# nmndeep/Robust-Segmentation

Measured on AMD Instinct MI355X. Metric: SEA attack-iterations/sec (UperNet-CNX-T, 512x512), higher is better.
Workload: dtype f32 (frozen-weight GEMMs on the 16-bit matrix cores by operand splitting: fp16x2 (22 significant bits per operand, 3 MFMA products) forward, fp16x2 (22 significant bits per operand, 3 MFMA products) input gradient; fp32 storage and accumulate)

## Files before the change

### devtools/gemm_big_stamps.py

```python
#!/usr/bin/env python3
import ctypes as C
import os
import subprocess
import sys

ROOT = os.path.dirname(os.path.dirname(os.path.abspath(__file__)))
PKG = os.path.join(ROOT, "robust-segmentation_amd")
SO = os.path.join(ROOT, "devtools", "_knock", "libbigdiag.so")

if "--build" in sys.argv:
    os.makedirs(os.path.dirname(SO), exist_ok=True)
    subprocess.run(["/opt/rocm/bin/hipcc", "-O3", "-fPIC", "-shared", "-std=c++17", "--offload-arch=gfx950", "-fno-slp-vectorize",
                    "-DSEA_GEMM_BIG_DIAG", os.path.join(PKG, "csrc", "gemm_split_big.hip"), "-o", SO], check=True)
    print(SO)
    sys.exit(0)

sys.path[:0] = [ROOT, PKG]
import numpy as np
import torch
from semseg import _native as N

args = [a for a in sys.argv[1:] if not a.startswith("-")]
G, M, K, Nn = [int(v) for v in (args[:4] if len(args) >= 4 else (36, 8192, 512, 512))]
STEPS = next(([int(v) for v in a[8:].split(",")] for a in sys.argv if a.startswith("--steps=")), [0, 93, 186, 372, 690])
L = C.CDLL(SO)
L.sea_gemm_big_diag.restype = C.c_int
L.sea_gemm_big_diag.argtypes = [C.c_void_p, C.c_int64, C.c_void_p, C.c_void_p, C.c_int64, C.c_int, C.c_int, C.c_int, C.c_int,
                                C.c_int64, C.c_int64, C.c_int64, C.c_void_p, C.c_int, C.c_int, C.c_int, C.c_void_p, C.c_void_p]
A = torch.randn(G, M, K, device="cuda")
W = torch.randn(G, Nn, K, device="cuda") / K ** 0.5
Wp = N.gemm_split_pack(W, terms=22)
out = torch.empty(G, M, Nn, device="cuda")
amax = torch.empty(M, dtype=torch.int32, device="cuda")
N.lib().sea_absmax_bits(N._p(A[0]), K, M, K, 1, 0, 1, N._p(amax), N._stream())
TILES = G * ((M + 255) // 256) * (Nn // 256)
stamps = torch.zeros(TILES, 8, dtype=torch.int64, device="cuda")
CUS = torch.cuda.get_device_properties(0).multi_processor_count


def launch(ko, step, st=None):
    rc = L.sea_gemm_big_diag(A.data_ptr(), K, Wp.data.data_ptr(), out.data_ptr(), Nn, M, Nn, K, G, M * K, Wp.stride, M * Nn,
                             amax.data_ptr(), 1, ko, step, st.data_ptr() if st is not None else None, N._stream())
    assert rc == 0, rc


def timed(ko, step, reps=20):
    launch(ko, step)
    torch.cuda.synchronize()
    e0, e1 = torch.cuda.Event(enable_timing=True), torch.cuda.Event(enable_timing=True)
    e0.record()
    for _ in range(reps):
        launch(ko, step)
    e1.record()
    torch.cuda.synchronize()
    return e0.elapsed_time(e1) / reps * 1e3


def us(ticks):
    return np.asarray(ticks, dtype=np.float64) / 100.0


def warm(seconds=2.0):
    import time
    t0 = time.perf_counter()
    while time.perf_counter() - t0 < seconds:
        for _ in range(50):
            launch(0, 0)
        torch.cuda.synchronize()


def stamp_table(ko, step):
    warm(0.5)
    for i in range(10):
        launch(ko, step, stamps if i == 5 else None)
    torch.cuda.synchronize()
    s = stamps.cpu().numpy().astype(np.int64)
    t = s[:, :6] - s[:, 0].min()
    cu = ((s[:, 6] >> 32) & 0xf) * 256 + ((s[:, 6] >> 8) & 0xff)
    seg = {"entry -> first load (stagger wait)": t[:, 1] - t[:, 0], "first load -> first MFMA (prologue)": t[:, 2] - t[:, 1],
           "K loop": t[:, 3] - t[:, 2], "K loop end -> last store issued": t[:, 4] - t[:, 3],
           "last store issued -> drained": t[:, 5] - t[:, 4], "whole block": t[:, 5] - t[:, 0]}
    print(f"\nko={ko} step={step} ticks: {len(np.unique(cu))} distinct CUs, launch span {us(t[:, 5].max()):.1f} us\n")
    print("| segment (wave 0) | median us | p10 | p90 |\n|---|---|---|---|")
    for name, v in seg.items():
        print(f"| {name} | {np.median(us(v)):.2f} | {np.percentile(us(v), 10):.2f} | {np.percentile(us(v), 90):.2f} |")
    gaps, rounds = [], {}
    for c in np.unique(cu):
        rows = t[cu == c]
        rows = rows[np.argsort(rows[:, 0])]
        gaps += list(rows[1:, 0] - rows[:-1, 5])
        for r, row in enumerate(rows):
            rounds.setdefault(r, []).append(row)
    g = us(gaps)
    print(f"| block end -> successor's entry, same CU | {np.median(g):.2f} | {np.percentile(g, 10):.2f} | {np.percentile(g, 90):.2f} |")
    print("\n| round on its CU | blocks | K-loop end: p10-p90 span over CUs, us | median block us | median K loop us | median K loop end -> stores issued us |\n|---|---|---|---|---|---|")
    for r in sorted(rounds):
        rows = np.array(rounds[r])
        if len(rows) < 16:
            continue
        e = us(rows[:, 3])
        print(f"| {r} | {len(rows)} | {np.percentile(e, 90) - np.percentile(e, 10):.1f} | {np.median(us(rows[:, 5] - rows[:, 0])):.1f} |"
              f" {np.median(us(rows[:, 3] - rows[:, 2])):.1f} | {np.median(us(rows[:, 4] - rows[:, 3])):.2f} |")


print(f"## G={G} M={M} K={K} N={Nn}: {TILES} tiles, {CUS} CUs, {K // 32} K steps, C = {G * M * Nn * 4 / 1e6:.0f} MB")
warm()
stamp_table(0, 0)
stamp_table(0, 186)
stamp_table(1, 0)
stamp_table(64, 0)
warm(0.5)
print("\n| 20 launches back to back, median [min - max] of five rounds taken in turn | full kernel us | non-temporal C stores us | no C stores us |\n|---|---|---|---|")
res = {(ko, step): [] for step in STEPS for ko in (0, 64, 1)}
for _ in range(5):
    for key in res:
        res[key].append(timed(*key))
for step in STEPS:
    cells = " | ".join(f"{np.median(res[ko, step]):.1f} [{min(res[ko, step]):.1f} - {max(res[ko, step]):.1f}]" for ko in (0, 64, 1))
    print(f"| stagger step {step} ticks (spread {step * 8 / 100:.1f} us) | {cells} |", flush=True)
```

### robust-segmentation_amd/csrc/gemm_split_big.hip

```cpp
#include "gemm_split.h"

namespace sea {

#ifdef SEA_GEMM_BIG_DIAG
struct BigDiag {
  int first_round, step_ticks;
  unsigned long long* stamps;
};
#define SEA_BIG_DIAG_PARAM , const BigDiag dg
#define SEA_BIG_DIAG_ARG , dg
#define SEA_BIG_STAMP(i) do { if constexpr (STAMP) { __builtin_amdgcn_sched_barrier(0); stamp[i] = __builtin_amdgcn_s_memrealtime(); __builtin_amdgcn_sched_barrier(0); } } while (0)
#else
#define SEA_BIG_DIAG_PARAM
#define SEA_BIG_DIAG_ARG
#define SEA_BIG_STAMP(i) do {} while (0)
#endif

template <bool F16, int WM, int WN, int TN, int PRO, int DEPTH, int KO = 0, bool STAMP = false>
__global__ __launch_bounds__(64 * WM * WN) void gemm_split_big_kernel(const GemmSplitArgs p SEA_BIG_DIAG_PARAM) {
  static_assert(WM * WN == 8, "eight waves, two per SIMD");
  constexpr int TERMS = 2;
  constexpr int MI = 2;
  constexpr int NT = 64 * WM * WN;
  constexpr int RP = NT / 8;
  constexpr int BM = 32 * MI * WM, WT = 32 * TN, BN = WT * WN;
  constexpr int IMG_A = BM * 64, IMG_W = BN * 64;
  constexpr int STAGE = TERMS * (IMG_A + IMG_W);
  constexpr int NA = BM / RP;
  constexpr int NWT = BN * 4 / NT, NW = TERMS * NWT;
  constexpr int SLOTS = 3 * MI * TN;
  constexpr int UNIT_EVERY = SLOTS / (3 * NA);
  constexpr bool HAS_T = (PRO == 1 || PRO == 3);
  static_assert(STAGE == 65536 && SLOTS % (3 * NA) == 0 && NW + 2 <= SLOTS, "configuration");
  extern __shared__ __attribute__((aligned(16))) char smem[];
  float* const row_sc = (float*)(smem + 2 * STAGE);
  float* const row_inv = row_sc + BM;

  const int M = p.M, N = p.N, K = p.K, Npad = p.Npad;
  const int64_t lda = p.lda, ldc = p.ldc;
  const int logical = (int)(blockIdx.x & 7) * p.per_xcd + (int)(blockIdx.x >> 3);
  if ((int)(blockIdx.x >> 3) >= p.per_xcd || logical >= p.total) return;
  const int nb = logical % p.nblocks;
  const int t2 = logical / p.nblocks;
  const int mb = t2 % p.mblocks;
  const int g = t2 / p.mblocks;
  const int m0 = mb * BM, n0 = nb * BN;
#ifdef SEA_GEMM_BIG_DIAG
  [[maybe_unused]] uint64_t stamp[6] = {};
  SEA_BIG_STAMP(0);
  if ((int)blockIdx.x < dg.first_round) {
    const uint32_t want = (uint32_t)(t2 % 8) * (uint32_t)dg.step_ticks;
    const uint32_t trips = (want >> 3) + 16;
    const uint64_t t0 = __builtin_amdgcn_s_memrealtime();
    for (uint32_t it = 0; it < trips && (uint32_t)(__builtin_amdgcn_s_memrealtime() - t0) < want; ++it) __builtin_amdgcn_s_sleep(8);
  }
  SEA_BIG_STAMP(1);
#endif
  const float* const w_inv = F16 ? (const float*)((const char*)p.w_inv + (int64_t)g * p.strideW) : nullptr;

  const int tid = threadIdx.x, lane = tid & 63, wave = tid >> 6;
  const int wm = wave / WN, wn = wave % WN;
  const int r = lane & 31, h = lane >> 5;
  const int q = tid & 7, arow = tid >> 3;

  const char* const Abase = (const char*)(p.A + (int64_t)g * p.strideA);
  const char* const Tbase = HAS_T ? (const char*)(p.a_gelu_grad_of + (int64_t)g * p.strideA) : nullptr;
  const float* const bias = p.bias;
  const int nkb = K / GS_BK;
  const char* const Wbase = p.W + (int64_t)g * p.strideW + (int64_t)n0 * 64;
  const int64_t w_term = (int64_t)Npad * 64, w_kb = (int64_t)TERMS * w_term;
  const uint32_t woff = (uint32_t)tid * 16;
  const uint32_t a_bytes = (uint32_t)((((int64_t)(M - 1)) * lda + K) * 4);
  const uint32_t w_bytes = (uint32_t)((int64_t)nkb * w_kb - (int64_t)n0 * 64);

  float a_sc[NA];
#pragma unroll
  for (int i = 0; i < NA; ++i) a_sc[i] = 1.f;
  const uint32_t aoff0 = (uint32_t)(((int64_t)(m0 + arow) * lda + 4 * q) * 4);
  const uint32_t a_wr0 = (uint32_t)(arow * 64 + swz<false>(arow, q >> 1) + (q & 1) * 8);
  const int wrow0 = tid >> 2;
  const uint32_t w_wr0 = (uint32_t)(TERMS * IMG_A + wrow0 * 64 + swz<false>(wrow0, tid & 3));
  const int a_row_step = (int)(RP * lda * 4);
  const int ra = wm * 32 * MI + r, rb = wn * WT + r;
  const uint32_t a_rd = (uint32_t)(ra * 64 + swz<false>(ra, h));
  const uint32_t b_rd = (uint32_t)(TERMS * IMG_A + rb * 64 + swz<false>(rb, h));

  struct Tile {
    f32x4 a[NA];
    f32x4 t[HAS_T ? NA : 1];
    u32x4 w[NW];
  };
  Tile R0 = {}, R1 = {};
  auto fetch_a = [&](Tile& R, int kb) __attribute__((always_inline)) {
    f32x4 (&Ra)[NA] = R.a;
    f32x4 (&Rt)[HAS_T ? NA : 1] = R.t;
    const int live = kb < nkb ? (int)a_bytes : 0;
    const __amdgpu_buffer_rsrc_t rs = __builtin_amdgcn_make_buffer_rsrc((void*)Abase, 0, live, 0x00020000);
#pragma unroll
    for (int i = 0; i < NA; ++i)
      Ra[i] = __builtin_bit_cast(f32x4, __builtin_amdgcn_raw_buffer_load_b128(
          rs, (int)((m0 + arow + RP * i < M) ? aoff0 : a_bytes), kb * (GS_BK * 4) + i * a_row_step, 0));
    if constexpr (HAS_T) {
      const __amdgpu_buffer_rsrc_t rt = __builtin_amdgcn_make_buffer_rsrc((void*)Tbase, 0, live, 0x00020000);
#pragma unroll
      for (int i = 0; i < NA; ++i)
        Rt[i] = __builtin_bit_cast(f32x4, __builtin_amdgcn_raw_buffer_load_b128(
            rt, (int)((m0 + arow + RP * i < M) ? aoff0 : a_bytes), kb * (GS_BK * 4) + i * a_row_step, 0));
    }
  };
  auto fetch_w = [&](Tile& R, int kb) __attribute__((always_inline)) {
    u32x4 (&Rw)[NW] = R.w;
    const __amdgpu_buffer_rsrc_t rs = __builtin_amdgcn_make_buffer_rsrc((void*)Wbase, 0, kb < nkb ? (int)w_bytes : 0, 0x00020000);
#pragma unroll
    for (int i = 0; i < NW; ++i)
      Rw[i] = __builtin_bit_cast(u32x4, __builtin_amdgcn_raw_buffer_load_b128(
                                            rs, (int)woff, kb * (int)w_kb + (i / NWT) * (int)w_term + (i % NWT) * (16 * NT), 0));
  };
  auto write_w = [&](Tile& R, int i, char* stage) __attribute__((always_inline)) {
    *(u32x4*)(stage + w_wr0 + (i / NWT) * IMG_W + (i % NWT) * (16 * NT)) = R.w[i];
  };

  f32x4 sv;
  uint32_t hi_a, hi_b;
  auto unit_a = [&](Tile& R, int i, int part, char* stage) __attribute__((always_inline)) {
    f32x4 (&Rt)[HAS_T ? NA : 1] = R.t;
    if (part == 0) {
      f32x4 v = R.a[i];
      if constexpr (PRO == 1) {
#pragma unroll
        for (int e = 0; e < 4; ++e) v[e] *= gelu_grad_f(Rt[i][e]);
      }
      if constexpr (PRO == 2) {
#pragma unroll
        for (int e = 0; e < 4; ++e) v[e] = gelu_f(v[e]);
      }
      if constexpr (PRO == 3) {
#pragma unroll
        for (int e = 0; e < 4; ++e) v[e] = Rt[i][e] > 0.f ? v[e] : 0.f;
      }
      if constexpr (F16) {
#pragma unroll
        for (int e = 0; e < 4; ++e) v[e] *= a_sc[i];
        hi_a = pack_f16(v[0], v[1]);
        hi_b = pack_f16(v[2], v[3]);
      } else {
        hi_a = pack_bf16(v[0], v[1]);
        hi_b = pack_bf16(v[2], v[3]);
      }
      sv = v;
    } else if (part == 1) {
      if constexpr (F16) {
        const f32x2 f0 = __builtin_convertvector(__builtin_bit_cast(f16x2, hi_a), f32x2);
        const f32x2 f1 = __builtin_convertvector(__builtin_bit_cast(f16x2, hi_b), f32x2);
        sv[0] -= f0[0];
        sv[1] -= f0[1];
        sv[2] -= f1[0];
        sv[3] -= f1[1];
      } else {
#pragma clang fp contract(off)
        sv[0] -= __uint_as_float(hi_a << 16);
        sv[1] -= __uint_as_float(hi_a & 0xffff0000u);
        sv[2] -= __uint_as_float(hi_b << 16);
        sv[3] -= __uint_as_float(hi_b & 0xffff0000u);
      }
    } else {
      *(u32x2*)(stage + a_wr0 + 64 * RP * i) = u32x2{hi_a, hi_b};
      const u32x2 mid = F16 ? u32x2{pack_f16(sv[0], sv[1]), pack_f16(sv[2], sv[3])}
                            : u32x2{pack_bf16(sv[0], sv[1]), pack_bf16(sv[2], sv[3])};
      *(u32x2*)(stage + IMG_A + a_wr0 + 64 * RP * i) = mid;
    }
  };

  bf16x8 fa[MI][TERMS], fb[TN][TERMS];
  auto read_a = [&](const char* stage, int s) __attribute__((always_inline)) {
#pragma unroll
    for (int mi = 0; mi < MI; ++mi)
#pragma unroll
      for (int t = 0; t < TERMS; ++t) fa[mi][t] = *(const bf16x8*)(stage + ((a_rd ^ (uint32_t)(32 * s)) + mi * 2048 + t * IMG_A));
  };
  auto read_b = [&](const char* stage, int s, int ni) __attribute__((always_inline)) {
#pragma unroll
    for (int t = 0; t < TERMS; ++t) fb[ni][t] = *(const bf16x8*)(stage + ((b_rd ^ (uint32_t)(32 * s)) + ni * 2048 + t * IMG_W));
  };
  auto mfma3 = [&](f32x16& c, int mi, int ni, int j) __attribute__((always_inline)) {
    const int ia = j == 0 ? 1 : 0, ib = j == 1 ? 1 : 0;
    if constexpr (F16)
      c = __builtin_amdgcn_mfma_f32_32x32x16_f16(__builtin_bit_cast(f16x8, fa[mi][ia]), __builtin_bit_cast(f16x8, fb[ni][ib]), c, 0, 0, 0);
    else
      c = __builtin_amdgcn_mfma_f32_32x32x16_bf16(fa[mi][ia], fb[ni][ib], c, 0, 0, 0);
  };

  f32x16 acc[MI][TN];
#pragma unroll
  for (int mi = 0; mi < MI; ++mi)
#pragma unroll
    for (int ni = 0; ni < TN; ++ni)
#pragma unroll
      for (int e = 0; e < 16; ++e) acc[mi][ni][e] = 0.f;

#define SEA_PIN() __builtin_amdgcn_sched_barrier(0)
  auto step = [&](char* cur, char* nxt, Tile& Rn, int kf) __attribute__((always_inline)) {
    int unit = 0;
    SEA_PIN();
#pragma unroll
    for (int ni = 0; ni < TN; ++ni) {
#pragma unroll
      for (int mi = 0; mi < MI; ++mi) {
#pragma unroll
        for (int j = 0; j < 3; ++j) {
          mfma3(acc[mi][ni], mi, ni, j);
          const int slot = (ni * MI + mi) * 3 + j;
          if (slot % UNIT_EVERY == 0 && unit < 3 * NA) {
            unit_a(Rn, unit / 3, unit % 3, nxt);
            ++unit;
          }
          SEA_PIN();
        }
      }
      read_b(cur, 1, ni);
      SEA_PIN();
    }
    read_a(cur, 1);
    SEA_PIN();
#pragma unroll
    for (int ni = 0; ni < TN; ++ni) {
#pragma unroll
      for (int mi = 0; mi < MI; ++mi) {
#pragma unroll
        for (int j = 0; j < 3; ++j) {
          mfma3(acc[mi][ni], mi, ni, j);
          const int slot = (ni * MI + mi) * 3 + j;
          if (slot < NW) write_w(Rn, slot < NW ? slot : 0, nxt);
          if (slot == NW) fetch_a(Rn, kf);
          if (slot == NW + 1) fetch_w(Rn, kf);
          SEA_PIN();
        }
      }
    }
    __syncthreads();
    read_a(nxt, 0);
#pragma unroll
    for (int ni = 0; ni < TN; ++ni) read_b(nxt, 0, ni);
    SEA_PIN();
  };

  char* const st0 = smem;
  char* const st1 = smem + STAGE;
  Tile& RA = R0;
  Tile& RB = DEPTH == 2 ? R1 : R0;
  fetch_a(R0, 0);
  fetch_w(R0, 0);
  if constexpr (DEPTH == 2) {
    fetch_a(R1, 1);
    fetch_w(R1, 1);
  }
  if constexpr (F16) {
    if (tid < BM) {
      int row = m0 + tid;
      row = row < M ? row : M - 1;
      float sc, inv;
      uint32_t word = p.amax_bits[p.amax_rows > 0 ? row / p.amax_rows : 0];
      const float mul = p.amax_mul_dev ? *p.amax_mul_dev : p.amax_mul;
      if (mul != 1.f) word = __float_as_uint(__uint_as_float(word) * mul) & 0x7fffffffu;
      pow2_scale(word, sc, inv);
      row_sc[tid] = sc;
      row_inv[tid] = inv;
    }
    __syncthreads();
#pragma unroll
    for (int i = 0; i < NA; ++i) a_sc[i] = row_sc[arow + RP * i];
  }
  SEA_PIN();
#pragma unroll
  for (int i = 0; i < NA; ++i) {
    unit_a(R0, i, 0, st0);
    unit_a(R0, i, 1, st0);
    unit_a(R0, i, 2, st0);
  }
#pragma unroll
  for (int i = 0; i < NW; ++i) write_w(R0, i, st0);
  fetch_a(R0, DEPTH);
  fetch_w(R0, DEPTH);
  __syncthreads();
  read_a(st0, 0);
#pragma unroll
  for (int ni = 0; ni < TN; ++ni) read_b(st0, 0, ni);
  SEA_BIG_STAMP(2);
  int kb = 0;
  for (; kb + 2 <= nkb; kb += 2) {
    step(st0, st1, RB, kb + 1 + DEPTH);
    step(st1, st0, RA, kb + 2 + DEPTH);
  }
  if (kb < nkb) step(st0, st1, RB, nkb);
#undef SEA_PIN
  SEA_BIG_STAMP(3);

  float bv_c[TN], wi_c[TN];
#pragma unroll
  for (int ni = 0; ni < TN; ++ni) {
    const int col = n0 + wn * WT + ni * 32 + r;
    bv_c[ni] = (bias && col < N) ? bias[col] : 0.f;
    wi_c[ni] = (F16 && col < N) ? w_inv[col] : 1.f;
  }
  const int wave_u = __builtin_amdgcn_readfirstlane(wave);
  const int row0_u = m0 + (wave_u / WN) * 32 * MI;
  float* const Cg = p.C + (int64_t)g * p.strideC;
  constexpr int SCR = 32 * WT * 4;
  char* const scr = smem + wave_u * SCR;
  constexpr int F4_ROW = WT / 4;
  const bool vec = (((ldc | p.strideC | N) & 3) == 0) && ((((uintptr_t)p.C) & 15) == 0);
  const int relu = p.relu;
  uint32_t omax = 0;
#pragma unroll
  for (int mi = 0; mi < MI; ++mi) {
    if (mi) asm volatile("s_waitcnt lgkmcnt(0)" ::: "memory");
    f32x4 ri[4] = {};
    if constexpr (F16) {
#pragma unroll
      for (int j = 0; j < 4; ++j) ri[j] = *(const f32x4*)(row_inv + (wave_u / WN) * 32 * MI + mi * 32 + 8 * j + 4 * h);
    }
#pragma unroll
    for (int ni = 0; ni < TN; ++ni) {
#pragma unroll
      for (int e = 0; e < 16; ++e) {
        const int row_l = (e & 3) + 8 * (e >> 2) + 4 * h;
        const float v = (F16 ? acc[mi][ni][e] * (ri[e >> 2][e & 3] * wi_c[ni]) : acc[mi][ni][e]) + bv_c[ni];
        *(float*)(scr + (row_l * WT + ni * 32 + r) * 4) = v;
      }
    }
    asm volatile("s_waitcnt lgkmcnt(0)" ::: "memory");
    constexpr int CH = WT / 16;
#pragma unroll
    for (int k0 = 0; k0 < WT / 8; k0 += CH) {
      f32x4 vv[CH];
#pragma unroll
      for (int j = 0; j < CH; ++j) vv[j] = *(const f32x4*)(scr + ((k0 + j) * 64 + lane) * 16);
#pragma unroll
      for (int j = 0; j < CH; ++j) {
        const int f = (k0 + j) * 64 + lane;
        const int row_l = f / F4_ROW, c4 = f - row_l * F4_ROW;
        f32x4 v = vv[j];
        const int row = row0_u + mi * 32 + row_l, col4 = n0 + wn * WT + 4 * c4;
        if (row >= M || col4 >= N) continue;
        float* const cp = Cg + (int64_t)row * ldc + col4;
        if (relu) {
#pragma unroll
          for (int e = 0; e < 4; ++e) v[e] = v[e] > 0.f ? v[e] : 0.f;
        }
        if constexpr ((KO & 1) != 0) {
          if (__float_as_uint(v[0]) != 0x7fc12345u) continue;
        }
        if (vec) {
          if constexpr ((KO & 64) != 0) __builtin_nontemporal_store(v, (f32x4*)cp);
          else *(f32x4*)cp = v;
        } else {
#pragma unroll
          for (int e = 0; e < 4; ++e)
            if (col4 + e < N) cp[e] = v[e];
        }
#pragma unroll
        for (int e = 0; e < 4; ++e) {
          const uint32_t vb = (col4 + e < N) ? (__float_as_uint(v[e]) & 0x7fffffffu) : 0u;
          omax = vb > omax ? vb : omax;
        }
      }
    }
  }
  if (p.out_amax != nullptr) {
#pragma unroll
    for (int o = 32; o > 0; o >>= 1) {
      const uint32_t other = (uint32_t)__shfl_xor((int)omax, o, 64);
      omax = other > omax ? other : omax;
    }
    if (lane == 0 && omax > *(volatile uint32_t*)p.out_amax) atomicMax(p.out_amax, omax);
  }
#ifdef SEA_GEMM_BIG_DIAG
  if constexpr (STAMP) {
    SEA_BIG_STAMP(4);
    asm volatile("s_waitcnt vmcnt(0)" ::: "memory");
    SEA_BIG_STAMP(5);
    if (tid == 0) {
      unsigned long long* const o = dg.stamps + (int64_t)logical * 8;
#pragma unroll
      for (int i = 0; i < 6; ++i) o[i] = stamp[i];
      o[6] = (unsigned long long)__builtin_amdgcn_s_getreg(4 | (31 << 11)) | ((unsigned long long)__builtin_amdgcn_s_getreg(20 | (31 << 11)) << 32);
      o[7] = blockIdx.x;
    }
  }
#endif
}

int gemm_split_big_launch(const GemmSplitArgs& p, const GemmPlan& pl, hipStream_t st) {
#ifdef SEA_GEMM_BIG_DIAG
  const BigDiag dg = {0, 0, nullptr};
#endif
  constexpr auto key = [](int wide, int f16, int pro, int depth) { return wide | f16 << 1 | pro << 2 | depth << 4; };
#define SEA_BIG_CASE(WIDE, F16, PRO, DEPTH)  \
  case key(WIDE, F16, PRO, DEPTH):           \
    gemm_launch<gemm_split_big_kernel<F16, WIDE ? 2 : 4, WIDE ? 4 : 2, WIDE ? 3 : 4, PRO, DEPTH>>(p, pl, st SEA_BIG_DIAG_ARG); \
    return 0;
#define SEA_BIG_MODES(F16) \
  SEA_BIG_CASE(0, F16, 0, 1) SEA_BIG_CASE(1, F16, 0, 2) SEA_BIG_CASE(1, F16, 1, 1) SEA_BIG_CASE(1, F16, 2, 2) SEA_BIG_CASE(1, F16, 3, 1)
  switch (key(pl.kernel == GEMM_BIG384, pl.f16, pl.pro, pl.depth)) {
    SEA_BIG_MODES(true)
    SEA_BIG_MODES(false)
  }
#undef SEA_BIG_MODES
#undef SEA_BIG_CASE
  return SEA_ERR_ARG;
}

#ifdef SEA_GEMM_BIG_DIAG
extern "C" int sea_gemm_big_diag(const float* A, int64_t lda, const void* Wp, float* C, int64_t ldc, int M, int N, int K, int batch,
                                 int64_t strideA, int64_t strideW_bytes, int64_t strideC, const uint32_t* amax_bits, int amax_rows,
                                 int ko, int step_ticks, unsigned long long* stamps, void* stream) {
  GemmPlan pl;
  if (gemm_plan(GemmQuery{M, N, K, 22, batch, lda, ldc, 0, 0, false, SEA_GEMM_PIPE_BIG}, &pl) != 0 || pl.kernel != GEMM_BIG256) return 1;
  const GemmSplitArgs p = gemm_args_init(pl, A, lda, Wp, C, ldc, M, N, K, strideA, strideW_bytes, strideC, amax_bits, amax_rows);
  int dev = 0, cus = 0;
  (void)hipGetDevice(&dev);
  if (hipDeviceGetAttribute(&cus, hipDeviceAttributeMultiprocessorCount, dev) != hipSuccess) return 1;
  BigDiag dg = {0, 0, stamps};
  if (step_ticks > 0 && step_ticks <= 1250 && p.total > cus) {
    dg.first_round = cus;
    dg.step_ticks = step_ticks;
  }
  const hipStream_t st = (hipStream_t)stream;
#define SEA_BIG_KO(KO, STAMP) gemm_launch<gemm_split_big_kernel<true, 4, 2, 4, 0, 1, KO, STAMP>>(p, pl, st, dg)
  if (ko == 0) { if (stamps) SEA_BIG_KO(0, true); else SEA_BIG_KO(0, false); }
  else if (ko == 1) { if (stamps) SEA_BIG_KO(1, true); else SEA_BIG_KO(1, false); }
  else if (ko == 64) { if (stamps) SEA_BIG_KO(64, true); else SEA_BIG_KO(64, false); }
  else return 1;
#undef SEA_BIG_KO
  return (int)hipGetLastError();
}
#endif

}
```

Measured before the change: 565.6.

## Move the stage barrier into the MFMA schedule and prefetch next-stage fragments early

The big split-GEMM K loop now places the __syncthreads partway through the second half-step and issues the next stage's LDS fragment reads (B columns and the first A row-block) as soon as their registers are released, rather than after a barrier at the end of each step. LDS addresses for both stages are precomputed into pinned VGPRs, so stage pointers become indices. The aim is to hide the barrier and LDS read latency behind the remaining MFMAs. The cost is more live address registers and a more intricate schedule, with a risk of register pressure or LDS hazards; a compile-time KL level (default 2) keeps the old path selectable, and the diagnostic script gains a K-loop comparison mode.

```diff
diff --git a/devtools/gemm_big_stamps.py b/devtools/gemm_big_stamps.py
--- a/devtools/gemm_big_stamps.py
+++ b/devtools/gemm_big_stamps.py
@@ -7,6 +7,7 @@
 ROOT = os.path.dirname(os.path.dirname(os.path.abspath(__file__)))
 PKG = os.path.join(ROOT, "robust-segmentation_amd")
 SO = os.path.join(ROOT, "devtools", "_knock", "libbigdiag.so")
+OTHER_SO = next((a[5:] for a in sys.argv if a.startswith("--so=")), None)
 
 if "--build" in sys.argv:
     os.makedirs(os.path.dirname(SO), exist_ok=True)
@@ -23,7 +24,7 @@
 args = [a for a in sys.argv[1:] if not a.startswith("-")]
 G, M, K, Nn = [int(v) for v in (args[:4] if len(args) >= 4 else (36, 8192, 512, 512))]
 STEPS = next(([int(v) for v in a[8:].split(",")] for a in sys.argv if a.startswith("--steps=")), [0, 93, 186, 372, 690])
-L = C.CDLL(SO)
+L = C.CDLL(OTHER_SO or SO)
 L.sea_gemm_big_diag.restype = C.c_int
 L.sea_gemm_big_diag.argtypes = [C.c_void_p, C.c_int64, C.c_void_p, C.c_void_p, C.c_int64, C.c_int, C.c_int, C.c_int, C.c_int,
                                 C.c_int64, C.c_int64, C.c_int64, C.c_void_p, C.c_int, C.c_int, C.c_int, C.c_void_p, C.c_void_p]
@@ -80,7 +81,9 @@
     seg = {"entry -> first load (stagger wait)": t[:, 1] - t[:, 0], "first load -> first MFMA (prologue)": t[:, 2] - t[:, 1],
            "K loop": t[:, 3] - t[:, 2], "K loop end -> last store issued": t[:, 4] - t[:, 3],
            "last store issued -> drained": t[:, 5] - t[:, 4], "whole block": t[:, 5] - t[:, 0]}
-    print(f"\nko={ko} step={step} ticks: {len(np.unique(cu))} distinct CUs, launch span {us(t[:, 5].max()):.1f} us\n")
+    kloop = np.median(us(seg["K loop"]))
+    print(f"\nko={ko} step={step} ticks: {len(np.unique(cu))} distinct CUs, launch span {us(t[:, 5].max()):.1f} us,"
+          f" K loop {kloop:.2f} us = {kloop / (K // 32):.3f} us per K step\n")
     print("| segment (wave 0) | median us | p10 | p90 |\n|---|---|---|---|")
     for name, v in seg.items():
         print(f"| {name} | {np.median(us(v)):.2f} | {np.percentile(us(v), 10):.2f} | {np.percentile(us(v), 90):.2f} |")
@@ -105,6 +108,20 @@
 
 print(f"## G={G} M={M} K={K} N={Nn}: {TILES} tiles, {CUS} CUs, {K // 32} K steps, C = {G * M * Nn * 4 / 1e6:.0f} MB")
 warm()
+if "--kloop" in sys.argv:
+    kos = [0] if OTHER_SO else [256, 257, 258]
+    print(f"library: {OTHER_SO or SO}; ko = 256 + KL")
+    for ko in kos:
+        stamp_table(ko, 0)
+    warm(0.5)
+    res = {ko: [] for ko in kos}
+    for _ in range(5):
+        for ko in kos:
+            res[ko].append(timed(ko, 0))
+    print("\n| 20 launches back to back, five rounds taken in turn | median us | min | max |\n|---|---|---|---|")
+    for ko in kos:
+        print(f"| ko={ko} | {np.median(res[ko]):.1f} | {min(res[ko]):.1f} | {max(res[ko]):.1f} |", flush=True)
+    sys.exit(0)
 stamp_table(0, 0)
 stamp_table(0, 186)
 stamp_table(1, 0)
diff --git a/robust-segmentation_amd/csrc/gemm_split_big.hip b/robust-segmentation_amd/csrc/gemm_split_big.hip
--- a/robust-segmentation_amd/csrc/gemm_split_big.hip
+++ b/robust-segmentation_amd/csrc/gemm_split_big.hip
@@ -15,8 +15,11 @@
 #define SEA_BIG_DIAG_ARG
 #define SEA_BIG_STAMP(i) do {} while (0)
 #endif
-
-template <bool F16, int WM, int WN, int TN, int PRO, int DEPTH, int KO = 0, bool STAMP = false>
+#ifndef SEA_BIG_KL
+#define SEA_BIG_KL 2
+#endif
+
+template <bool F16, int WM, int WN, int TN, int PRO, int DEPTH, int KO = 0, bool STAMP = false, int KL = SEA_BIG_KL>
 __global__ __launch_bounds__(64 * WM * WN) void gemm_split_big_kernel(const GemmSplitArgs p SEA_BIG_DIAG_PARAM) {
   static_assert(WM * WN == 8, "eight waves, two per SIMD");
   constexpr int TERMS = 2;
@@ -84,6 +87,19 @@
   const int ra = wm * 32 * MI + r, rb = wn * WT + r;
   const uint32_t a_rd = (uint32_t)(ra * 64 + swz<false>(ra, h));
   const uint32_t b_rd = (uint32_t)(TERMS * IMG_A + rb * 64 + swz<false>(rb, h));
+  uint32_t a_rdx[2][2], b_rdx[2][2], a_wrx[2], w_wrx[2];
+#pragma unroll
+  for (int st = 0; st < 2; ++st) {
+#pragma unroll
+    for (int s = 0; s < 2; ++s) {
+      a_rdx[st][s] = (uint32_t)(st * STAGE) + (a_rd ^ (uint32_t)(32 * s));
+      b_rdx[st][s] = (uint32_t)(st * STAGE) + (b_rd ^ (uint32_t)(32 * s));
+      asm volatile("" : "+v"(a_rdx[st][s]), "+v"(b_rdx[st][s]));
+    }
+    a_wrx[st] = (uint32_t)(st * STAGE) + a_wr0;
+    w_wrx[st] = (uint32_t)(st * STAGE) + w_wr0;
+    asm volatile("" : "+v"(a_wrx[st]), "+v"(w_wrx[st]));
+  }
 
   struct Tile {
     f32x4 a[NA];
@@ -116,13 +132,13 @@
       Rw[i] = __builtin_bit_cast(u32x4, __builtin_amdgcn_raw_buffer_load_b128(
                                             rs, (int)woff, kb * (int)w_kb + (i / NWT) * (int)w_term + (i % NWT) * (16 * NT), 0));
   };
-  auto write_w = [&](Tile& R, int i, char* stage) __attribute__((always_inline)) {
-    *(u32x4*)(stage + w_wr0 + (i / NWT) * IMG_W + (i % NWT) * (16 * NT)) = R.w[i];
+  auto write_w = [&](Tile& R, int i, int st) __attribute__((always_inline)) {
+    *(u32x4*)(smem + w_wrx[st] + ((i / NWT) * IMG_W + (i % NWT) * (16 * NT))) = R.w[i];
   };
 
   f32x4 sv;
   uint32_t hi_a, hi_b;
-  auto unit_a = [&](Tile& R, int i, int part, char* stage) __attribute__((always_inline)) {
+  auto unit_a = [&](Tile& R, int i, int part, int st) __attribute__((always_inline)) {
     f32x4 (&Rt)[HAS_T ? NA : 1] = R.t;
     if (part == 0) {
       f32x4 v = R.a[i];
@@ -164,23 +180,21 @@
         sv[3] -= __uint_as_float(hi_b & 0xffff0000u);
       }
     } else {
-      *(u32x2*)(stage + a_wr0 + 64 * RP * i) = u32x2{hi_a, hi_b};
+      *(u32x2*)(smem + a_wrx[st] + 64 * RP * i) = u32x2{hi_a, hi_b};
       const u32x2 mid = F16 ? u32x2{pack_f16(sv[0], sv[1]), pack_f16(sv[2], sv[3])}
                             : u32x2{pack_bf16(sv[0], sv[1]), pack_bf16(sv[2], sv[3])};
-      *(u32x2*)(stage + IMG_A + a_wr0 + 64 * RP * i) = mid;
+      *(u32x2*)(smem + a_wrx[st] + (IMG_A + 64 * RP * i)) = mid;
     }
   };
 
   bf16x8 fa[MI][TERMS], fb[TN][TERMS];
-  auto read_a = [&](const char* stage, int s) __attribute__((always_inline)) {
-#pragma unroll
-    for (int mi = 0; mi < MI; ++mi)
-#pragma unroll
-      for (int t = 0; t < TERMS; ++t) fa[mi][t] = *(const bf16x8*)(stage + ((a_rd ^ (uint32_t)(32 * s)) + mi * 2048 + t * IMG_A));
-  };
-  auto read_b = [&](const char* stage, int s, int ni) __attribute__((always_inline)) {
-#pragma unroll
-    for (int t = 0; t < TERMS; ++t) fb[ni][t] = *(const bf16x8*)(stage + ((b_rd ^ (uint32_t)(32 * s)) + ni * 2048 + t * IMG_W));
+  auto read_a = [&](int st, int s, int mi) __attribute__((always_inline)) {
+#pragma unroll
+    for (int t = 0; t < TERMS; ++t) fa[mi][t] = *(const bf16x8*)(smem + a_rdx[st][s] + (mi * 2048 + t * IMG_A));
+  };
+  auto read_b = [&](int st, int s, int ni) __attribute__((always_inline)) {
+#pragma unroll
+    for (int t = 0; t < TERMS; ++t) fb[ni][t] = *(const bf16x8*)(smem + b_rdx[st][s] + (ni * 2048 + t * IMG_W));
   };
   auto mfma3 = [&](f32x16& c, int mi, int ni, int j) __attribute__((always_inline)) {
     const int ia = j == 0 ? 1 : 0, ib = j == 1 ? 1 : 0;
@@ -199,7 +213,10 @@
       for (int e = 0; e < 16; ++e) acc[mi][ni][e] = 0.f;
 
 #define SEA_PIN() __builtin_amdgcn_sched_barrier(0)
-  auto step = [&](char* cur, char* nxt, Tile& Rn, int kf) __attribute__((always_inline)) {
+  constexpr int BAR = NW + 1, COL = 3 * MI, A0_FREE = (TN - 1) * COL + 2;
+  static_assert(BAR <= A0_FREE, "the barrier stands before the last column releases fa[0]");
+  auto step = [&](const int cur, Tile& Rn, int kf, const bool last) __attribute__((always_inline)) {
+    const int nxt = cur ^ 1;
     int unit = 0;
     SEA_PIN();
 #pragma unroll
@@ -214,13 +231,15 @@
             unit_a(Rn, unit / 3, unit % 3, nxt);
             ++unit;
           }
+          if (KL >= 2 && slot == A0_FREE) read_a(cur, 1, 0);
           SEA_PIN();
         }
       }
       read_b(cur, 1, ni);
       SEA_PIN();
     }
-    read_a(cur, 1);
+    if (KL < 2) read_a(cur, 1, 0);
+    read_a(cur, 1, 1);
     SEA_PIN();
 #pragma unroll
     for (int ni = 0; ni < TN; ++ni) {
@@ -233,19 +252,32 @@
           if (slot < NW) write_w(Rn, slot < NW ? slot : 0, nxt);
           if (slot == NW) fetch_a(Rn, kf);
           if (slot == NW + 1) fetch_w(Rn, kf);
+          if constexpr (KL >= 1) {
+            if (slot == BAR) __syncthreads();
+            if (slot >= BAR && !last) {
+#pragma unroll
+              for (int c = 0; c + 1 < TN; ++c)
+                if (c * COL + COL - 1 == slot || (slot == BAR && c * COL + COL - 1 < BAR)) read_b(nxt, 0, c);
+              if (slot == A0_FREE) read_a(nxt, 0, 0);
+            }
+          }
           SEA_PIN();
         }
       }
     }
-    __syncthreads();
-    read_a(nxt, 0);
-#pragma unroll
-    for (int ni = 0; ni < TN; ++ni) read_b(nxt, 0, ni);
+    if constexpr (KL == 0) {
+      __syncthreads();
+      read_a(nxt, 0, 0);
+      read_a(nxt, 0, 1);
+#pragma unroll
+      for (int ni = 0; ni < TN; ++ni) read_b(nxt, 0, ni);
+    } else if (!last) {
+      read_a(nxt, 0, 1);
+      read_b(nxt, 0, TN - 1);
+    }
     SEA_PIN();
   };
 
-  char* const st0 = smem;
-  char* const st1 = smem + STAGE;
   Tile& RA = R0;
   Tile& RB = DEPTH == 2 ? R1 : R0;
   fetch_a(R0, 0);
@@ -273,25 +305,26 @@
   SEA_PIN();
 #pragma unroll
   for (int i = 0; i < NA; ++i) {
-    unit_a(R0, i, 0, st0);
-    unit_a(R0, i, 1, st0);
-    unit_a(R0, i, 2, st0);
-  }
-#pragma unroll
-  for (int i = 0; i < NW; ++i) write_w(R0, i, st0);
+    unit_a(R0, i, 0, 0);
+    unit_a(R0, i, 1, 0);
+    unit_a(R0, i, 2, 0);
+  }
+#pragma unroll
+  for (int i = 0; i < NW; ++i) write_w(R0, i, 0);
   fetch_a(R0, DEPTH);
   fetch_w(R0, DEPTH);
   __syncthreads();
-  read_a(st0, 0);
-#pragma unroll
-  for (int ni = 0; ni < TN; ++ni) read_b(st0, 0, ni);
+#pragma unroll
+  for (int mi = 0; mi < MI; ++mi) read_a(0, 0, mi);
+#pragma unroll
+  for (int ni = 0; ni < TN; ++ni) read_b(0, 0, ni);
   SEA_BIG_STAMP(2);
   int kb = 0;
   for (; kb + 2 <= nkb; kb += 2) {
-    step(st0, st1, RB, kb + 1 + DEPTH);
-    step(st1, st0, RA, kb + 2 + DEPTH);
-  }
-  if (kb < nkb) step(st0, st1, RB, nkb);
+    step(0, RB, kb + 1 + DEPTH, false);
+    step(1, RA, kb + 2 + DEPTH, false);
+  }
+  if (kb < nkb) step(0, RB, nkb, true);
 #undef SEA_PIN
   SEA_BIG_STAMP(3);
 
@@ -426,10 +459,13 @@
     dg.step_ticks = step_ticks;
   }
   const hipStream_t st = (hipStream_t)stream;
-#define SEA_BIG_KO(KO, STAMP) gemm_launch<gemm_split_big_kernel<true, 4, 2, 4, 0, 1, KO, STAMP>>(p, pl, st, dg)
-  if (ko == 0) { if (stamps) SEA_BIG_KO(0, true); else SEA_BIG_KO(0, false); }
-  else if (ko == 1) { if (stamps) SEA_BIG_KO(1, true); else SEA_BIG_KO(1, false); }
-  else if (ko == 64) { if (stamps) SEA_BIG_KO(64, true); else SEA_BIG_KO(64, false); }
+#define SEA_BIG_KO(KO, STAMP, KL) gemm_launch<gemm_split_big_kernel<true, 4, 2, 4, 0, 1, KO, STAMP, KL>>(p, pl, st, dg)
+  if (ko == 0) { if (stamps) SEA_BIG_KO(0, true, SEA_BIG_KL); else SEA_BIG_KO(0, false, SEA_BIG_KL); }
+  else if (ko == 1) { if (stamps) SEA_BIG_KO(1, true, SEA_BIG_KL); else SEA_BIG_KO(1, false, SEA_BIG_KL); }
+  else if (ko == 64) { if (stamps) SEA_BIG_KO(64, true, SEA_BIG_KL); else SEA_BIG_KO(64, false, SEA_BIG_KL); }
+  else if (ko == 256) { if (stamps) SEA_BIG_KO(0, true, 0); else SEA_BIG_KO(0, false, 0); }
+  else if (ko == 257) { if (stamps) SEA_BIG_KO(0, true, 1); else SEA_BIG_KO(0, false, 1); }
+  else if (ko == 258) { if (stamps) SEA_BIG_KO(0, true, 2); else SEA_BIG_KO(0, false, 2); }
   else return 1;
 #undef SEA_BIG_KO
   return (int)hipGetLastError();
```

After: 570.0, median of 6. Within noise of the previous version (+0.8%).
